# jihun1998/AO

Measured on AMD Instinct MI355X. Metric: points/sec fwd+bwd PTv2m2 S3DIS, higher is better.
Workload: dtype fp32

## Files before the change

### ao_amd/csrc/common.h

```cpp
#pragma once
#include <hip/hip_runtime.h>
#include <stdint.h>
#include <stdlib.h>

#include "../../include/ptv2_hip.h"

#define WAVE 64

#define PTV2_CHECK_LAUNCH()                         \
    do {                                            \
        if (hipGetLastError() != hipSuccess) return PTV2_ERR_LAUNCH; \
    } while (0)

#define RUN(call)                        \
    do {                                 \
        int rc_ = (call);                \
        if (rc_ != PTV2_OK) return rc_;  \
    } while (0)

static inline int divup(long long a, long long b) { return (int)((a + b - 1) / b); }

static constexpr size_t ptv2_align256(size_t v) { return (v + 255) & ~(size_t)255; }
struct PtvCarver {
    char *p; size_t off;
    char *take(size_t bytes) { char *r = p ? p + off : nullptr; off += ptv2_align256(bytes); return r; }
    template <class T> T *take_n(size_t count) { return (T *)take(sizeof(T) * count); }
};

static inline bool ptv2_env_set(const char *name) { return getenv(name) != nullptr; }
static inline bool ptv2_env_is(const char *name, char c) { const char *e = getenv(name); return e && e[0] == c; }

enum PtvKernelId {
    KID_KNN_QUERY = 0, KID_LOGITS_FWD, KID_SOFTMAX_ROWS, KID_AGG_TILE, KID_PEB_FWD, KID_PEB_BWD, KID_BWD_TILE,
    KID_BWD_ROWS, KID_BWD_GV, KID_LOGITS_BWD_ROWS, KID_LOGITS_BWD_GATHER, KID_LOGITS_BWD_PARAMS, KID_WGRAD,
    KID_BN_STATS, KID_BN_APPLY, KID_BN_BWD_REDUCE, KID_BN_BWD_APPLY, KID_SKINNY_FWD, KID_SKINNY_BWD, KID_ROWS_GEMM,  KID_BWD_POINT = KID_ROWS_GEMM + 8,
     KID_WGRAD_LDS = KID_BWD_POINT + 5 ,
    KID_WGRAD_GROUPED ,
    KID_FWD_POINT ,
    KID_LOGITS_BWD_FUSED ,
    KID_BN_BWD_APPLY_RES = KID_LOGITS_BWD_FUSED + 5 ,
    KID_BN_BWD_FINAPPLY ,
    KID_FWD_TILE ,
    KID_WGRAD_TILE = KID_FWD_TILE + 4 ,
    KID_BWD_TILE_K ,
    KID_AUG_POINTS = KID_BWD_TILE_K + 4 ,
    KID_COUNT
};
extern "C" int ptv2_profile_is_on(void);
int ptv2_profile_wants(int kid);
void ptv2_profile_begin(int kid, hipStream_t st);
void ptv2_profile_end(int kid, hipStream_t st, double algorithmic_bytes);
struct PtvScopedTimer {
    int kid; hipStream_t st; double bytes; bool on;
    PtvScopedTimer(int k, hipStream_t s, double b) : kid(k), st(s), bytes(b), on(ptv2_profile_wants(k) != 0) {
        if (on) ptv2_profile_begin(kid, st);
    }
    ~PtvScopedTimer() { if (on) ptv2_profile_end(kid, st, bytes); }
};

enum PtvGraphSlot { GRAPH_MODEL_FWD = 0, GRAPH_MODEL_BWD = 1, GRAPH_MODEL_FWD_PREFIX = 2, GRAPH_MODEL_FWD_REST = 3, GRAPH_SLOTS = 4 };
struct PtvGraphScope {
    void *st, *cap; int which, ring_entry; bool active; long long t0;
    PtvGraphScope(void *stream, int which, bool allow = true);
    void *stream() const { return cap; }
    int finish(int rc);
    ~PtvGraphScope();
    PtvGraphScope(const PtvGraphScope &) = delete;
    PtvGraphScope &operator=(const PtvGraphScope &) = delete;
};
int ptv2_graph_capturing(void);
int ptv2_profile_stamps(void);
int ptv2_zero_async(void *p, size_t bytes, hipStream_t st);

void ptv2_wgrad_defer_begin(void *arena, size_t bytes);
bool ptv2_wgrad_defer_active();
float *ptv2_wgrad_defer_alloc(size_t floats);
void ptv2_wgrad_defer_arm(bool on);
void ptv2_wgrad_defer_arm_rs(bool on);
bool ptv2_wgrad_defer_armed_rs();
struct PtvWgradArm {
    explicit PtvWgradArm(bool on) { ptv2_wgrad_defer_arm(on); }
    ~PtvWgradArm() { ptv2_wgrad_defer_arm(false); }
    PtvWgradArm(const PtvWgradArm &) = delete;
    PtvWgradArm &operator=(const PtvWgradArm &) = delete;
};
struct PtvWgradArmRs {
    explicit PtvWgradArmRs(bool on) { ptv2_wgrad_defer_arm_rs(on); }
    ~PtvWgradArmRs() { ptv2_wgrad_defer_arm_rs(false); }
    PtvWgradArmRs(const PtvWgradArmRs &) = delete;
    PtvWgradArmRs &operator=(const PtvWgradArmRs &) = delete;
};
int ptv2_wgrad_defer_flush(void *stream);
void ptv2_wgrad_defer_end();
size_t ptv2_wgrad_defer_table_bytes();

int ptv2_matmul_bf16(void);
void ptv2_set_matmul_bf16(int on);
struct PtvMatmulScope {
    int prev;
    explicit PtvMatmulScope(int on) : prev(ptv2_matmul_bf16()) { ptv2_set_matmul_bf16(on); }
    ~PtvMatmulScope() { ptv2_set_matmul_bf16(prev); }
};
typedef __bf16 ptv2_bf16x8 __attribute__((ext_vector_type(8)));
__device__ __forceinline__ ptv2_bf16x8 ptv2_pack_bf16(float4 lo, float4 hi) {
    ptv2_bf16x8 r;
    r[0] = (__bf16)lo.x; r[1] = (__bf16)lo.y; r[2] = (__bf16)lo.z; r[3] = (__bf16)lo.w;
    r[4] = (__bf16)hi.x; r[5] = (__bf16)hi.y; r[6] = (__bf16)hi.z; r[7] = (__bf16)hi.w;
    return r;
}

static __device__ __attribute__((aligned(16), unused)) float ptv2_zero_pad[1024];
template <class T>
__device__ __forceinline__ T ptv2_ld_or_zero(const T *p, bool ok) {
    return *(ok ? p : (const T *)ptv2_zero_pad);
}

#define PTV2_NUM_COUNTERS 64
enum PtvCounterSlot { CNT_LOGITS_FWD = 0, CNT_BP2, CNT_LOGITS_BWD_ROWS, CNT_CE, CNT_LOVASZ, CNT_BN_TILES = 16  };
unsigned *ptv2_stream_counters(hipStream_t st);

__device__ __forceinline__ float ref_d2(float qx, float qy, float qz, float x, float y, float z) {
    float dx = qx - x, dy = qy - y, dz = qz - z;
    return __builtin_fmaf(dz, dz, __builtin_fmaf(dx, dx, dy * dy));
}

__device__ __forceinline__ int seg_of(int pt, const int *__restrict__ offset, int b) {
    int lo = 0, hi = b - 1;
    while (lo < hi) {
        int mid = (lo + hi) >> 1;
        if (pt < offset[mid]) hi = mid; else lo = mid + 1;
    }
    return lo;
}

__device__ __forceinline__ int f2ord(float f) {
    int i = __float_as_int(f);
    return i >= 0 ? i : i ^ 0x7fffffff;
}
__device__ __forceinline__ float ord2f(int i) {
    return __int_as_float(i >= 0 ? i : i ^ 0x7fffffff);
}

__device__ __forceinline__ unsigned long long shfl_xor_u64(unsigned long long v, int m) {
    unsigned lo = (unsigned)v, hi = (unsigned)(v >> 32);
    lo = __shfl_xor(lo, m, WAVE);
    hi = __shfl_xor(hi, m, WAVE);
    return ((unsigned long long)hi << 32) | lo;
}

__device__ __forceinline__ int xcd_remap(int orig, int nwg) {
    int q = nwg >> 3, r = nwg & 7, x = orig & 7;
    return (x < r ? x * (q + 1) : r * (q + 1) + (x - r) * q) + (orig >> 3);
}
// ... 3 lines not shown
```

### ao_amd/csrc/graph.hip

```cpp
#include <algorithm>
#include <atomic>
#include <chrono>
#include <cstdio>
#include <cstdlib>
#include <mutex>
#include <unordered_map>

#include "common.h"

namespace {

struct SlotKey {
    int device;
    hipStream_t stream;
    int which;
    bool operator==(const SlotKey &o) const { return device == o.device && stream == o.stream && which == o.which; }
};
struct SlotKeyHash {
    size_t operator()(const SlotKey &k) const {
        return std::hash<void *>()((void *)k.stream) * 131u + (size_t)k.device * 7u + (size_t)k.which;
    }
};
constexpr int RING = 8;
struct Exec {
    hipGraphExec_t exec = nullptr;
    size_t nodes = 0;
    hipEvent_t done = nullptr;
    bool in_flight = false;
    unsigned long long seq = 0;
};
struct Slot {
    Exec ring[RING];
    unsigned long long launches = 0;
};
int pick_entry(Slot &slot) {
    int oldest = 0;
    for (int i = 0; i < RING; ++i) {
        Exec &e = slot.ring[i];
        if (e.in_flight && e.done && hipEventQuery(e.done) == hipSuccess) e.in_flight = false;
        if (!e.in_flight) return i;
        if (e.seq < slot.ring[oldest].seq) oldest = i;
    }
    (void)hipGetLastError();
    return oldest;
}
struct StreamKey {
    int device;
    hipStream_t stream;
    bool operator==(const StreamKey &o) const { return device == o.device && stream == o.stream; }
};
struct StreamKeyHash {
    size_t operator()(const StreamKey &k) const { return std::hash<void *>()((void *)k.stream) * 131u + (size_t)k.device; }
};
std::unordered_map<StreamKey, hipStream_t, StreamKeyHash> g_capture_streams;

std::mutex g_mu;
std::unordered_map<SlotKey, Slot, SlotKeyHash> g_slots;
std::unordered_map<StreamKey, hipEvent_t, StreamKeyHash> g_last_done;
std::atomic<int> g_mode{-1};
thread_local int g_inside = 0;

struct Stats {
    std::atomic<long long> scopes{0}, updated{0}, instantiated{0}, declined{0}, nodes{0};
    std::atomic<long long> capture_ns{0}, update_ns{0}, launch_ns{0}, wait_ns{0};
} g_stats;

long long now_ns() {
    return std::chrono::duration_cast<std::chrono::nanoseconds>(std::chrono::steady_clock::now().time_since_epoch()).count();
}

int mode() {
    int m = g_mode.load(std::memory_order_relaxed);
    if (m < 0) {
        m = ptv2_env_is("AO_AMD_GRAPH", '0') ? 0 : 1;
        g_mode.store(m, std::memory_order_relaxed);
    }
    return m;
}

}

int ptv2_graph_capturing(void) { return g_inside; }

namespace {
__global__ __launch_bounds__(256) void zero_kernel(float4 *__restrict__ p, long long n4, float *__restrict__ tail, int ntail) {
    const float4 z = make_float4(0.f, 0.f, 0.f, 0.f);
    for (long long i = (long long)blockIdx.x * 256 + threadIdx.x; i < n4; i += (long long)gridDim.x * 256) p[i] = z;
    if (blockIdx.x == 0 && (int)threadIdx.x < ntail) tail[threadIdx.x] = 0.f;
}
}

int ptv2_zero_async(void *p, size_t bytes, hipStream_t st) {
    if (bytes == 0) return PTV2_OK;
    if (!p || (bytes & 3) || ((uintptr_t)p & 15)) return PTV2_ERR_ARG;
    const long long n4 = (long long)(bytes >> 4);
    const int ntail = (int)((bytes & 15) >> 2);
    const int grid = (int)std::min<long long>(std::max<long long>((n4 + 255) / 256, 1), 2048);
    hipLaunchKernelGGL(zero_kernel, dim3(grid), dim3(256), 0, st, (float4 *)p, n4, (float *)p + 4 * n4, ntail);
    return PTV2_OK;
}

extern "C" int ptv2_graph_mode(int on) {
    const int prev = mode();
    if (on >= 0) g_mode.store(on ? 1 : 0, std::memory_order_relaxed);
    return prev;
}

extern "C" int ptv2_graph_stats(double *out, int reset) {
    if (out) {
        out[0] = (double)g_stats.scopes.load(); out[1] = (double)g_stats.updated.load();
        out[2] = (double)g_stats.instantiated.load(); out[3] = (double)g_stats.declined.load();
        out[4] = (double)g_stats.nodes.load(); out[5] = 1e-3 * (double)g_stats.capture_ns.load();
        out[6] = 1e-3 * (double)g_stats.update_ns.load(); out[7] = 1e-3 * (double)g_stats.launch_ns.load();
        out[8] = 1e-3 * (double)g_stats.wait_ns.load();
    }
    if (reset) {
        g_stats.scopes = 0; g_stats.updated = 0; g_stats.instantiated = 0; g_stats.declined = 0; g_stats.nodes = 0;
        g_stats.capture_ns = 0; g_stats.update_ns = 0; g_stats.launch_ns = 0; g_stats.wait_ns = 0;
    }
    return PTV2_OK;
}

extern "C" int ptv2_graph_reset(void) {
    std::lock_guard<std::mutex> lk(g_mu);
    for (auto &kv : g_slots)
        for (Exec &e : kv.second.ring) {
            if (e.in_flight && e.done) (void)hipEventSynchronize(e.done);
            if (e.exec) (void)hipGraphExecDestroy(e.exec);
            if (e.done) (void)hipEventDestroy(e.done);
        }
    g_slots.clear();
    g_last_done.clear();
    for (auto &kv : g_capture_streams) (void)hipStreamDestroy(kv.second);
    g_capture_streams.clear();
    return PTV2_OK;
}

PtvGraphScope::PtvGraphScope(void *stream, int which_, bool allow)
    : st(stream), cap(stream), which(which_), ring_entry(0), active(false), t0(0) {
    hipStream_t s = (hipStream_t)stream;
    if (!allow || !mode() || g_inside) { g_stats.declined++; return; }
    if (ptv2_profile_is_on() && !ptv2_profile_stamps()) { g_stats.declined++; return; }
    hipStreamCaptureStatus cs = hipStreamCaptureStatusNone;
    if (s != nullptr && (hipStreamIsCapturing(s, &cs) != hipSuccess || cs != hipStreamCaptureStatusNone)) {
        g_stats.declined++; (void)hipGetLastError(); return;
    }
    int device = 0;
    if (hipGetDevice(&device) != hipSuccess) { g_stats.declined++; return; }
    if (which == GRAPH_MODEL_FWD_PREFIX || which == GRAPH_MODEL_FWD) {
        if (!ptv2_env_is("AO_AMD_GRAPH_IDLE_EAGER", '0')) {
            hipEvent_t last = nullptr;
            {
                std::lock_guard<std::mutex> lk(g_mu);
                auto it = g_last_done.find(StreamKey{device, s});
                if (it != g_last_done.end()) last = it->second;
            }
            if (last && hipEventQuery(last) == hipSuccess) return;
            (void)hipGetLastError();
        }
    }
    hipStream_t c = nullptr;
    {
        std::lock_guard<std::mutex> lk(g_mu);
        auto it = g_capture_streams.find(StreamKey{device, s});
        if (it != g_capture_streams.end()) {
            c = it->second;
        } else {
            if (hipStreamCreateWithFlags(&c, hipStreamNonBlocking) != hipSuccess) { g_stats.declined++; (void)hipGetLastError(); return; }
            if (!ptv2_stream_counters(c) || hipStreamSynchronize(c) != hipSuccess) {
                (void)hipStreamDestroy(c); g_stats.declined++; return;
            }
            g_capture_streams[StreamKey{device, s}] = c;
        }
    }
    int entry = 0;
    {
        std::lock_guard<std::mutex> lk(g_mu);
        entry = pick_entry(g_slots[SlotKey{device, s, which}]);
    }
    t0 = now_ns();
    if (hipStreamBeginCapture(c, hipStreamCaptureModeRelaxed) != hipSuccess) { g_stats.declined++; (void)hipGetLastError(); return; }
    cap = (void *)c;
    active = true;
    g_inside = 1;
    g_stats.scopes++;
    ring_entry = entry;
    ptv2_profile_scope(which, 0, entry, RING);
}

int PtvGraphScope::finish(int rc) {
    if (!active) return rc;
    active = false;
    ptv2_profile_scope(which, 1, 0, RING);
    g_inside = 0;
    hipStream_t s = (hipStream_t)st;
    hipGraph_t g = nullptr;
    const hipError_t ec = hipStreamEndCapture((hipStream_t)cap, &g);
    const long long t1 = now_ns();
    g_stats.capture_ns += t1 - t0;
    if (ec != hipSuccess || !g) { (void)hipGetLastError(); if (g) (void)hipGraphDestroy(g); return rc != PTV2_OK ? rc : PTV2_ERR_LAUNCH; }
    if (rc != PTV2_OK) { (void)hipGraphDestroy(g); return rc; }
    int device = 0;
    (void)hipGetDevice(&device);
    size_t nodes = 0;
    (void)hipGraphGetNodes(g, nullptr, &nodes);
    int out = PTV2_OK;
    Exec *slot_p = nullptr;
    Slot *ring_p = nullptr;
    {
        std::lock_guard<std::mutex> lk(g_mu);
        Slot &ring = g_slots[SlotKey{device, s, which}];
        ring_p = &ring;
        slot_p = &ring.ring[ring_entry];
        slot_p->seq = ++ring.launches;
    }
    {
        Exec &slot = *slot_p;
        if (!slot.done && hipEventCreateWithFlags(&slot.done, hipEventDisableTiming | hipEventBlockingSync) != hipSuccess) slot.done = nullptr;
        if (slot.in_flight && slot.done) {
            const long long w0 = now_ns();
            (void)hipEventSynchronize(slot.done);
            g_stats.wait_ns += now_ns() - w0;
            slot.in_flight = false;
        }
        {
            static const int lead = [] { const char *e = getenv("AO_AMD_GRAPH_LEAD"); const int v = e ? atoi(e) : RING; return v < 1 ? 1 : (v > RING ? RING : v); }();
            if (lead < RING) {
                for (;;) {
                    int inflight = 0; Exec *oldest = nullptr;
                    for (int e2 = 0; e2 < RING; ++e2) {
                        Exec &o = ring_p->ring[e2];
                        if (&o == &slot || !o.in_flight || !o.done) continue;
                        if (hipEventQuery(o.done) == hipSuccess) { o.in_flight = false; continue; }
                        ++inflight;
                        if (!oldest || o.seq < oldest->seq) oldest = &o;
                    }
                    (void)hipGetLastError();
                    if (inflight < lead || !oldest) break;
                    const long long w0 = now_ns();
                    (void)hipEventSynchronize(oldest->done);
                    g_stats.wait_ns += now_ns() - w0;
                    oldest->in_flight = false;
                }
            }
        }
        const long long t1b = now_ns();
        bool ready = false;
        static const bool debug = ptv2_env_is("AO_AMD_GRAPH_DEBUG", '1');
        if (slot.exec && slot.nodes == nodes) {
            hipGraphExecUpdateResult res = hipGraphExecUpdateSuccess;
            hipGraphNode_t bad = nullptr;
            const hipError_t eu = hipGraphExecUpdate(slot.exec, g, &bad, &res);
            if (eu == hipSuccess && res == hipGraphExecUpdateSuccess) {
                ready = true;
                g_stats.updated++;
            } else {
                (void)hipGetLastError();
                if (debug) fprintf(stderr, "ptv2 graph: slot %d update failed rc %d result %d (%zu nodes)\n", which, (int)eu, (int)res, nodes);
            }
        } else if (debug && slot.exec) {
            fprintf(stderr, "ptv2 graph: slot %d node count %zu -> %zu\n", which, slot.nodes, nodes);
        }
        if (!ready) {
            if (slot.exec) { (void)hipGraphExecDestroy(slot.exec); slot.exec = nullptr; }
            if (hipGraphInstantiate(&slot.exec, g, nullptr, nullptr, 0) != hipSuccess) {
                (void)hipGetLastError();
                slot.exec = nullptr;
                out = PTV2_ERR_LAUNCH;
            } else {
                slot.nodes = nodes;
                g_stats.instantiated++;
                if (!ptv2_profile_is_on()) {
                    for (int e = 0; e < RING; ++e) {
                        Exec &o = ring_p->ring[e];
                        if (&o == &slot || o.exec || o.in_flight) continue;
                        if (hipGraphInstantiate(&o.exec, g, nullptr, nullptr, 0) != hipSuccess) { (void)hipGetLastError(); o.exec = nullptr; break; }
                        o.nodes = nodes;
                    }
                }
            }
        }
        const long long t2 = now_ns();
        g_stats.update_ns += t2 - t1b;
        if (out == PTV2_OK) {
            if (hipGraphLaunch(slot.exec, s) != hipSuccess) { (void)hipGetLastError(); out = PTV2_ERR_LAUNCH; }
            else if (slot.done && hipEventRecord(slot.done, s) == hipSuccess) {
                slot.in_flight = true;
                std::lock_guard<std::mutex> lk(g_mu);
                g_last_done[StreamKey{device, s}] = slot.done;
            }
            else if (hipStreamSynchronize(s) != hipSuccess) out = PTV2_ERR_LAUNCH;
            g_stats.launch_ns += now_ns() - t2;
            g_stats.nodes += (long long)nodes;
        }
    }
    (void)hipGraphDestroy(g);
    return out;
}

PtvGraphScope::~PtvGraphScope() {
    if (!active) return;
    ptv2_profile_scope(which, 1, 0, RING);
    g_inside = 0;
    hipGraph_t g = nullptr;
    (void)hipStreamEndCapture((hipStream_t)cap, &g);
    if (g) (void)hipGraphDestroy(g);
    (void)hipGetLastError();
}
```

### ao_amd/csrc/wgrad.hip

```cpp
#include <vector>

#include "dense_common.h"
#include "wgrad_job.h"

namespace dense {

using f32x4 = __attribute__((ext_vector_type(4))) float;
constexpr int WG_MT = 3, WG_TILE = 16 * WG_MT, WG_CHUNK = 256, WG_CHUNK_MIN = 128;

template <bool BF16>
__device__ __forceinline__ void wgrad_direct_tile(const int n, const int cout, const int cin, const int tiles_i,
                                                  const float *__restrict__ A, const long long ldy,
                                                  const float *__restrict__ B, const long long ldx, float *__restrict__ part,
                                                  const bool part_b, const int batch, const float *__restrict__ xs,
                                                  const float *__restrict__ xh, const int chunk, const int bx, const int by,
                                                  const int bz) {
    __shared__ float sRed[TPB / WAVE][WG_MT * WG_MT * 4 + WG_MT][WAVE + 1];
    const int lane = threadIdx.x & 63, wid = threadIdx.x >> 6;
    const int to = (by / tiles_i) * WG_TILE, ti = (by % tiles_i) * WG_TILE;
    const long long r0 = (long long)bx * chunk;
    const long long r1 = (r0 + chunk) < (long long)n ? (r0 + chunk) : (long long)n;
    const int lr = lane >> 4, lc = lane & 15;
    f32x4 acc[WG_MT][WG_MT];
    float bsum[WG_MT];
#pragma unroll
    for (int m = 0; m < WG_MT; ++m) {
        bsum[m] = 0.f;
#pragma unroll
        for (int t = 0; t < WG_MT; ++t) acc[m][t] = (f32x4){0.f, 0.f, 0.f, 0.f};
    }
    bool mo[WG_MT], mi[WG_MT];
    float xsc_[WG_MT], xsh_[WG_MT];
#pragma unroll
    for (int m = 0; m < WG_MT; ++m) {
        mo[m] = to + m * 16 + lc < cout;
        mi[m] = ti + m * 16 + lc < cin;
        xsc_[m] = (xs && mi[m]) ? xs[ti + m * 16 + lc] : 1.f;
        xsh_[m] = (xs && mi[m]) ? xh[ti + m * 16 + lc] : 0.f;
    }
    constexpr int U = 8;
    for (long long rb = r0 + 4 * wid; rb < r1; rb += 4 * (TPB / WAVE) * U) {
        float a[U][WG_MT], b[U][WG_MT];
#pragma unroll
        for (int u = 0; u < U; ++u) {
            const long long row = rb + (long long)u * 4 * (TPB / WAVE) + lr;
            const bool rok = row < r1;
#pragma unroll
            for (int m = 0; m < WG_MT; ++m) {
                a[u][m] = (rok && mo[m]) ? A[row * ldy + to + m * 16 + lc] : 0.f;
                b[u][m] = (rok && mi[m]) ? B[row * ldx + ti + m * 16 + lc] : 0.f;
            }
        }
        if (xs) {
#pragma unroll
            for (int u = 0; u < U; ++u)
#pragma unroll
                for (int m = 0; m < WG_MT; ++m) b[u][m] = fmaxf(__builtin_fmaf(b[u][m], xsc_[m], xsh_[m]), 0.f);
        }
        if constexpr (BF16) {
            ptv2_bf16x8 ab[WG_MT], bb[WG_MT];
#pragma unroll
            for (int m = 0; m < WG_MT; ++m) {
#pragma unroll
                for (int u = 0; u < U; ++u) {
                    bsum[m] += a[u][m];
                    ab[m][u] = (__bf16)a[u][m];
                    bb[m][u] = (__bf16)b[u][m];
                }
            }
#pragma unroll
            for (int m = 0; m < WG_MT; ++m)
#pragma unroll
                for (int t = 0; t < WG_MT; ++t)
                    acc[m][t] = __builtin_amdgcn_mfma_f32_16x16x32_bf16(ab[m], bb[t], acc[m][t], 0, 0, 0);
        } else {
#pragma unroll
            for (int u = 0; u < U; ++u)
#pragma unroll
                for (int m = 0; m < WG_MT; ++m) {
                    bsum[m] += a[u][m];
#pragma unroll
                    for (int t = 0; t < WG_MT; ++t)
// ... 116 lines not shown
    stash(0);
    __syncthreads();
    int buf = 0;
    for (long long rs = r0; rs < r1; rs += WL_ROWS, buf ^= 1) {
        const bool more = rs + WL_ROWS < r1;
        if (more) fetch(rs + WL_ROWS);
        const float *pa = sA + (size_t)buf * WL_ROWS * WG_TILE + (size_t)(wid * 16 + lr) * WG_TILE + lc;
        const float *pb = sB + (size_t)buf * WL_ROWS * WG_TILE + (size_t)(wid * 16 + lr) * WG_TILE + lc;
#pragma unroll
        for (int ks = 0; ks < 4; ++ks) {
            float a[WG_MT], b[WG_MT];
#pragma unroll
            for (int m = 0; m < WG_MT; ++m) {
                a[m] = pa[ks * 4 * WG_TILE + m * 16];
                b[m] = pb[ks * 4 * WG_TILE + m * 16];
            }
            if (xs) {
#pragma unroll
                for (int m = 0; m < WG_MT; ++m) b[m] = fmaxf(__builtin_fmaf(b[m], xsc_[m], xsh_[m]), 0.f);
            }
#pragma unroll
            for (int m = 0; m < WG_MT; ++m) {
                if constexpr (RS != 0) bsum[m] = __builtin_fmaf(a[m], sc_[ks], bsum[m]);
                else bsum[m] += a[m];
#pragma unroll
                for (int t = 0; t < WG_MT; ++t) acc[m][t] = __builtin_amdgcn_mfma_f32_16x16x4f32(a[m], b[t], acc[m][t], 0, 0, 0);
            }
        }
        if (more) {
            stash(buf ^ 1);
            __syncthreads();
        }
    }
    __syncthreads();
    float(*sRed)[WG_MT * WG_MT * 4 + WG_MT][WAVE + 1] = (float(*)[WG_MT * WG_MT * 4 + WG_MT][WAVE + 1]) wl_lds4;
#pragma unroll
    for (int m = 0; m < WG_MT; ++m) {
        float bs = bsum[m];
        bs += __shfl_xor(bs, 16, WAVE);
        bs += __shfl_xor(bs, 32, WAVE);
        sRed[wid][WG_MT * WG_MT * 4 + m][lane] = bs;
#pragma unroll
        for (int t = 0; t < WG_MT; ++t)
#pragma unroll
            for (int r = 0; r < 4; ++r) sRed[wid][(m * WG_MT + t) * 4 + r][lane] = acc[m][t][r];
    }
    __syncthreads();
    const size_t rec = (size_t)batch * cout * cin + (part_b ? (size_t)batch * cout : 0);
    float *p = part + (size_t)bx * rec + (size_t)bz * cout * cin;
    for (int e = threadIdx.x; e < WG_MT * WG_MT * 4 * WAVE; e += TPB) {
        const int q = e / WAVE, l = e - q * WAVE;
        const int mt = q / 4, r = q - mt * 4, m = mt / WG_MT, t = mt - m * WG_MT;
        const int o = to + m * 16 + (l >> 4) * 4 + r, i = ti + t * 16 + (l & 15);
        if (o < cout && i < cin) {
            float v = 0.f;
#pragma unroll
            for (int wv = 0; wv < TPB / WAVE; ++wv) v += sRed[wv][q][l];
            p[(size_t)o * cin + i] = v;
        }
    }
    if (part_b && ti == 0 && threadIdx.x < WG_TILE) {
        const int m = threadIdx.x >> 4, l = threadIdx.x & 15, o = to + threadIdx.x;
        if (o < cout) {
            float v = 0.f;
#pragma unroll
            for (int wv = 0; wv < TPB / WAVE; ++wv) v += sRed[wv][WG_MT * WG_MT * 4 + m][l];
            part[(size_t)bx * rec + (size_t)batch * cout * cin + (size_t)bz * cout + o] = v;
        }
    }
}

template <int RS>
__device__ __forceinline__ void wgrad_lds_job(const WgradJob &J, const int bx, const int by, const int bz) {
    const bool multi = J.count > 0;
    wgrad_lds_tile<RS>(J.n, J.cout, J.cin, J.tiles_i, multi ? J.mgY[bz] : J.gY + (long long)bz * J.sy, J.ldy,
                       multi ? J.mX[bz] : J.X + (long long)bz * J.sx, J.ldx, J.part, J.has_pb != 0, J.batch,
                       multi ? J.mxsc[bz] : nullptr, multi ? J.mxsh[bz] : nullptr, J.chunk, J.rowscale, J.lds_s, bx, by, bz);
}
template <int RS>
__global__ __launch_bounds__(TPB) void linear_wgrad_lds_kernel(WgradJob J) {
    wgrad_lds_job<RS>(J, (int)blockIdx.x, (int)blockIdx.y, (int)blockIdx.z);
}

constexpr int WGRAD_PACK = 8;
struct WgradJobPack { WgradJob j[WGRAD_PACK]; };
static_assert(sizeof(WgradJobPack) + 16 <= 4096, "the table writer's argument block must fit the 4 KB kernarg segment");
__global__ void wgrad_jobs_write_kernel(WgradJobPack pack, int count, WgradJob *table) {
    if ((int)threadIdx.x < count) table[threadIdx.x] = pack.j[threadIdx.x];
}

template <int RS>
__global__ __launch_bounds__(TPB) void linear_wgrad_lds_kernel_jobs(const WgradJob *__restrict__ jobs, int njobs) {
    int j = 0;
    while (j + 1 < njobs && (int)blockIdx.x >= jobs[j + 1].wg0) ++j;
    const WgradJob &J = jobs[j];
    const int local = (int)blockIdx.x - J.wg0;
    const int rest = local / J.chunks;
    wgrad_lds_job<RS>(J, local % J.chunks, rest % J.tiles, rest / J.tiles);
}

constexpr int GRP_I = 8;
__device__ __forceinline__ void grouped_wgrad_tile(const int n, const int c, const int g, const int gw, const int chunk,
                                                   const float *__restrict__ gY, const float *__restrict__ X,
                                                   const float *__restrict__ sw, float *__restrict__ part, const int rec,
                                                   const int bx, const int bg) {
    extern __shared__ float4 grp_lds4[];
    const int q = c >> 2, units = gw * q, R = max(1, TPB / units);
    const int tid = threadIdx.x, rs = tid / units, u = tid - rs * units;
    const bool active = rs < R;
    const int gl = u / q, qi = u - gl * q, grp = bg * gw + gl;
    const bool live = active && grp < g;
    float4 acc[GRP_I];
    float bacc[GRP_I];
#pragma unroll
    for (int i = 0; i < GRP_I; ++i) { acc[i] = make_float4(0.f, 0.f, 0.f, 0.f); bacc[i] = 0.f; }
    const long long r0 = (long long)bx * chunk, r1 = (r0 + chunk) < (long long)n ? (r0 + chunk) : (long long)n;
    if (live) {
        const float *xa = X + (size_t)grp * c + 4 * qi;
        const float *ya = gY + (size_t)grp * GRP_I;
        const float *sa = sw + grp;
        const size_t xs = (size_t)g * c;
        constexpr int U = 4;
        long long r = r0 + rs;
        for (; r + (long long)(U - 1) * R < r1; r += (long long)U * R) {
            float4 a[U], y0[U], y1[U];
            float s[U];
#pragma unroll
            for (int t = 0; t < U; ++t) {
                const size_t rr = (size_t)(r + (long long)t * R);
                a[t] = *(const float4 *)(xa + rr * xs);
                y0[t] = *(const float4 *)(ya + rr * c);
                y1[t] = *(const float4 *)(ya + rr * c + 4);
                s[t] = qi == 0 ? sa[rr * g] : 0.f;
            }
#pragma unroll
            for (int t = 0; t < U; ++t) {
                const float y[GRP_I] = {y0[t].x, y0[t].y, y0[t].z, y0[t].w, y1[t].x, y1[t].y, y1[t].z, y1[t].w};
#pragma unroll
                for (int i = 0; i < GRP_I; ++i) {
                    acc[i].x = __builtin_fmaf(y[i], a[t].x, acc[i].x); acc[i].y = __builtin_fmaf(y[i], a[t].y, acc[i].y);
                    acc[i].z = __builtin_fmaf(y[i], a[t].z, acc[i].z); acc[i].w = __builtin_fmaf(y[i], a[t].w, acc[i].w);
                    bacc[i] = __builtin_fmaf(y[i], s[t], bacc[i]);
                }
            }
        }
        for (; r < r1; r += R) {
            const size_t rr = (size_t)r;
            const float4 a = *(const float4 *)(xa + rr * xs), y0 = *(const float4 *)(ya + rr * c), y1 = *(const float4 *)(ya + rr * c + 4);
            const float sv = qi == 0 ? sa[rr * g] : 0.f;
            const float y[GRP_I] = {y0.x, y0.y, y0.z, y0.w, y1.x, y1.y, y1.z, y1.w};
#pragma unroll
            for (int i = 0; i < GRP_I; ++i) {
                acc[i].x = __builtin_fmaf(y[i], a.x, acc[i].x); acc[i].y = __builtin_fmaf(y[i], a.y, acc[i].y);
                acc[i].z = __builtin_fmaf(y[i], a.z, acc[i].z); acc[i].w = __builtin_fmaf(y[i], a.w, acc[i].w);
                bacc[i] = __builtin_fmaf(y[i], sv, bacc[i]);
            }
        }
    }
    float4 *sAcc = grp_lds4;
    float *sB = (float *)(sAcc + (size_t)R * GRP_I * units);
    if (active) {
#pragma unroll
        for (int i = 0; i < GRP_I; ++i) {
            sAcc[((size_t)rs * GRP_I + i) * units + u] = acc[i];
            if (qi == 0) sB[((size_t)rs * GRP_I + i) * gw + gl] = bacc[i];
        }
    }
    __syncthreads();
    if (rs == 0 && grp < g) {
        float *p = part + (size_t)bx * rec;
#pragma unroll
        for (int i = 0; i < GRP_I; ++i) {
            float4 v = sAcc[(size_t)i * units + u];
            for (int t = 1; t < R; ++t) {
                const float4 w = sAcc[((size_t)t * GRP_I + i) * units + u];
                v.x += w.x; v.y += w.y; v.z += w.z; v.w += w.w;
            }
            *(float4 *)(p + ((size_t)grp * GRP_I + i) * c + 4 * qi) = v;
            if (qi == 0) {
                float b = sB[(size_t)i * gw + gl];
                for (int t = 1; t < R; ++t) b += sB[((size_t)t * GRP_I + i) * gw + gl];
                p[(size_t)g * GRP_I * c + (size_t)grp * GRP_I + i] = b;
            }
        }
    }
}
inline size_t grouped_lds_bytes(int c, int gw) {
    const int units = gw * (c >> 2), R = std::max(1, TPB / units);
    return sizeof(float4) * (size_t)R * GRP_I * units + sizeof(float) * (size_t)R * GRP_I * gw;
}
__global__ __launch_bounds__(TPB) void grouped_wgrad_kernel(WgradJob J) {
    const int bx = (int)blockIdx.x % J.chunks, bg = (int)blockIdx.x / J.chunks;
    grouped_wgrad_tile(J.n, J.cin, J.batch, J.gw, J.chunk, J.gY, J.X, J.rowscale, J.part, J.rec, bx, bg);
}
__global__ __launch_bounds__(TPB) void grouped_wgrad_kernel_jobs(const WgradJob *__restrict__ jobs, int njobs) {
    int j = 0;
    while (j + 1 < njobs && (int)blockIdx.x >= jobs[j + 1].wg0) ++j;
    const WgradJob &J = jobs[j];
    const int local = (int)blockIdx.x - J.wg0;
    grouped_wgrad_tile(J.n, J.cin, J.batch, J.gw, J.chunk, J.gY, J.X, J.rowscale, J.part, J.rec, local % J.chunks, local / J.chunks);
}

template <bool BF16>
__global__ __launch_bounds__(TPB) void linear_wgrad_kernel_jobs(const WgradJob *__restrict__ jobs, int njobs) {
    int j = 0;
    while (j + 1 < njobs && (int)blockIdx.x >= jobs[j + 1].wg0) ++j;
    const WgradJob &J = jobs[j];
    const int local = (int)blockIdx.x - J.wg0;
    const int rest = local / J.chunks;
    wgrad_direct_job<BF16>(J, local % J.chunks, rest % J.tiles, rest / J.tiles);
}

__global__ __launch_bounds__(256) void wgrad_jobs_finalize_kernel(const WgradJob *__restrict__ jobs, int njobs, int total) {
    __shared__ double s_sum[3][64];
    const int sidx = blockIdx.x * 256 + threadIdx.x;
    int j = 0;
    while (j + 1 < njobs && (int)blockIdx.x * 256 >= jobs[j + 1].fin0) ++j;
    const WgradJob &J = jobs[j];
    const int lanes = J.fin_lanes, local = sidx - J.fin0;
    const int rg = lanes == 1 ? 0 : (int)threadIdx.x >> 6;
    const int col = lanes == 1 ? local : (local >> 8) * 64 + ((int)threadIdx.x & 63);
    const int nblk = J.chunks;
    const size_t len = (size_t)J.rec;
    const float *part = J.part;
    const bool ok = col < J.rec;
    double a0 = 0.0, a1 = 0.0, a2 = 0.0, a3 = 0.0;
    if (ok) {
        int b = rg;
        for (; b + 3 * lanes < nblk; b += 4 * lanes) {
            a0 += (double)part[(size_t)b * len + col];
            a1 += (double)part[(size_t)(b + lanes) * len + col];
            a2 += (double)part[(size_t)(b + 2 * lanes) * len + col];
            a3 += (double)part[(size_t)(b + 3 * lanes) * len + col];
        }
        for (; b < nblk; b += lanes) a0 += (double)part[(size_t)b * len + col];
    }
    double acc = (a0 + a1) + (a2 + a3);
    if (lanes != 1) {
        if (rg > 0) s_sum[rg - 1][threadIdx.x & 63] = acc;
        __syncthreads();
        if (rg > 0) return;
        acc = (acc + s_sum[0][threadIdx.x]) + (s_sum[1][threadIdx.x] + s_sum[2][threadIdx.x]);
    }
    if (!ok) return;
    const float v = (float)acc;
    const int wlen = J.cout * J.cin, wtot = J.batch * wlen;
    if (J.count > 0) {
        if (col < wtot) {
            const int p = col / wlen;
            J.mdW[p][col - p * wlen] = v;
        } else {
            const int r = col - wtot, p = r / J.cout;
            if (J.mdb[p]) J.mdb[p][r - p * J.cout] = v;
        }
    } else if (col < wtot) {
        J.dW[col] = v;
    } else if (J.db) {
        J.db[col - wtot] = v;
    }
}

static bool wgrad_lds_ok(const void *a, long long ldy, long long sy, const void *b, long long ldx, long long sx) {
    return ((uintptr_t)a % 16 == 0) && ((uintptr_t)b % 16 == 0) && ldy % 4 == 0 && ldx % 4 == 0 && sy % 4 == 0 && sx % 4 == 0;
}
static bool wgrad_lds_shape_ok(int cout, int cin) { return cout % 4 == 0 && cin % 4 == 0; }
constexpr size_t WL_LDS_BYTES = sizeof(float) * std::max<size_t>(4 * (size_t)WL_ROWS * WG_TILE,
                                                                 (size_t)(TPB / WAVE) * (WG_MT * WG_MT * 4 + WG_MT) * (WAVE + 1));

}

using namespace dense;

extern "C" size_t dense_workspace_bytes(int n, int cout, int cin) {
    const size_t chunks = (size_t)(n + WG_CHUNK_MIN - 1) / WG_CHUNK_MIN + 1;
    const size_t wg = sizeof(float) * chunks * ((size_t)cout * cin + cout);
    const size_t bn = sizeof(float) * (size_t)MAX_BLK * 2 * (size_t)std::max(cout, cin);
    return ptv2_align256(std::max(wg, bn)) + 1024;
}

static int wg_chunk(int n, int tiles, bool filed = false) {
    const int target = filed ? 256 : 768;
    const int chunks = std::max(1, target / std::max(1, tiles));
    const long long rows = ((long long)n + chunks - 1) / chunks;
    long long chunk = std::max<long long>(WG_CHUNK, (rows + 127) / 128 * 128);
    if (tiles > 1) {
        int guard = 0;
        while ((((long long)n + chunk - 1) / chunk) % 8 == 0 && ((long long)n + chunk - 1) / chunk > 1 && guard++ < 16) chunk += 128;
    }
    return (int)std::min<long long>(chunk, 1 << 20);
}

namespace {
enum WgradForm { WF_LDS = 0, WF_LDS_RS, WF_DIRECT, WF_DIRECT_BF16, WF_GROUPED, WF_RECOMPUTE, WGRAD_FORMS };
constexpr int wgrad_kid(WgradForm f) {
    return f == WF_RECOMPUTE ? KID_WGRAD_TILE : f == WF_GROUPED ? KID_WGRAD_GROUPED : (f == WF_LDS || f == WF_LDS_RS) ? KID_WGRAD_LDS : KID_WGRAD;
}
struct WgradCall {
    WgradJob J;
    WgradForm form;
    double bytes;
    size_t posrel;
};

struct WgradDefer {
    bool active = false;
    bool armed = false;
    bool armed_rs = false;
    char *arena = nullptr;
    size_t cap = 0, used = 0;
    std::vector<WgradJob> jobs[WGRAD_FORMS];
    double bytes[WGRAD_FORMS] = {};
};
thread_local WgradDefer g_wdefer;
constexpr int WGRAD_MAX_JOBS = 64;
constexpr size_t WGRAD_TABLE_BYTES = ptv2_align256(sizeof(WgradJob) * WGRAD_MAX_JOBS);

bool may_file(bool rs) { return g_wdefer.active && (rs ? g_wdefer.armed_rs : g_wdefer.armed); }

bool wgrad_configure() {
    static const bool ok = [] {
        const void *kernels[4] = {(const void *)linear_wgrad_lds_kernel<0>, (const void *)linear_wgrad_lds_kernel<1>,
                                  (const void *)linear_wgrad_lds_kernel_jobs<0>, (const void *)linear_wgrad_lds_kernel_jobs<1>};
        bool all = true;
        for (const void *k : kernels)
            all = hipFuncSetAttribute(k, hipFuncAttributeMaxDynamicSharedMemorySize, (int)WL_LDS_BYTES) == hipSuccess && all;
        return all;
    }();
    return ok;
}
}

void ptv2_wgrad_defer_begin(void *arena, size_t bytes) {
    WgradDefer &D = g_wdefer;
    for (int f = 0; f < WGRAD_FORMS; ++f) { D.jobs[f].clear(); D.bytes[f] = 0.0; }
    D.armed = D.armed_rs = false;
    D.active = arena != nullptr && bytes > WGRAD_FORMS * WGRAD_TABLE_BYTES;
    D.arena = (char *)arena;
    D.cap = bytes;
    D.used = WGRAD_FORMS * WGRAD_TABLE_BYTES;
}
bool ptv2_wgrad_defer_active() { return g_wdefer.active; }
void ptv2_wgrad_defer_end() {
    g_wdefer.active = g_wdefer.armed = g_wdefer.armed_rs = false;
    for (auto &j : g_wdefer.jobs) j.clear();
}
void ptv2_wgrad_defer_arm(bool on) { g_wdefer.armed = on && g_wdefer.active; }
void ptv2_wgrad_defer_arm_rs(bool on) { g_wdefer.armed_rs = on && g_wdefer.active; }
bool ptv2_wgrad_defer_armed_rs() { return may_file(true); }
size_t ptv2_wgrad_defer_table_bytes() { return WGRAD_FORMS * WGRAD_TABLE_BYTES; }
float *ptv2_wgrad_defer_alloc(size_t floats) {
    WgradDefer &D = g_wdefer;
    const size_t bytes = ptv2_align256(sizeof(float) * floats);
    if (!D.active || D.used + bytes > D.cap) return nullptr;
    float *p = (float *)(D.arena + D.used);
    D.used += bytes;
    return p;
}
int ptv2_wgrad_defer_flush(void *stream) {
    WgradDefer &D = g_wdefer;
    if (!D.active) return PTV2_OK;
    hipStream_t st = (hipStream_t)stream;
    if (!wgrad_configure()) return PTV2_ERR_LAUNCH;
    for (int f = 0; f < WGRAD_FORMS; ++f) {
        const WgradForm form = (WgradForm)f;
        std::vector<WgradJob> &jobs = D.jobs[form];
        if (jobs.empty()) continue;
        WgradJob *table = (WgradJob *)(D.arena + (size_t)form * WGRAD_TABLE_BYTES);
        const int njobs = (int)jobs.size();
        const bool row_pieces = form == WF_GROUPED || form == WF_RECOMPUTE;
        std::stable_sort(jobs.begin(), jobs.end(), [row_pieces](const WgradJob &a, const WgradJob &b) {
            const long long wa = (long long)a.chunk * (row_pieces ? a.gw * a.cin : 1), wb = (long long)b.chunk * (row_pieces ? b.gw * b.cin : 1);
            return wa > wb;
        });
        int wgs = 0, fin = 0;
        long long pos_wgs = 0;
        bool pos_all = form == WF_RECOMPUTE;
        for (WgradJob &J : jobs) {
            if (form == WF_RECOMPUTE) {
                J.ldy = pos_wgs;
                pos_wgs += ((long long)J.n * 16 + 255) / 256;
                pos_all = pos_all && J.mX[0] != nullptr;
            }
            J.wg0 = wgs; J.fin0 = fin;
            J.fin_lanes = J.chunks > 32 ? 4 : 1;
            wgs += J.wgs;
            fin += J.fin_lanes == 1 ? (J.rec + 255) / 256 * 256 : (J.rec + 63) / 64 * 256;
        }
        for (int at = 0; at < njobs; at += WGRAD_PACK) {
            WgradJobPack pack;
            const int cnt = std::min(WGRAD_PACK, njobs - at);
            for (int i = 0; i < WGRAD_PACK; ++i) pack.j[i] = jobs[(size_t)std::min(at + i, njobs - 1)];
            hipLaunchKernelGGL(wgrad_jobs_write_kernel, dim3(1), dim3(64), 0, st, pack, cnt, table + at);
        }
        {
            PtvScopedTimer t(wgrad_kid(form), st, D.bytes[form]);
            const dim3 grid((unsigned)wgs), block(TPB);
            const WgradJob *tab = table;
            switch (form) {
                case WF_LDS: hipLaunchKernelGGL(linear_wgrad_lds_kernel_jobs<0>, grid, block, WL_LDS_BYTES, st, tab, njobs); break;
                case WF_LDS_RS: hipLaunchKernelGGL(linear_wgrad_lds_kernel_jobs<1>, grid, block, WL_LDS_BYTES, st, tab, njobs); break;
                case WF_DIRECT: hipLaunchKernelGGL(linear_wgrad_kernel_jobs<false>, grid, block, 0, st, tab, njobs); break;
                case WF_DIRECT_BF16: hipLaunchKernelGGL(linear_wgrad_kernel_jobs<true>, grid, block, 0, st, tab, njobs); break;
                case WF_GROUPED: {
                    size_t lds = 0;
                    for (const WgradJob &J : jobs) lds = std::max(lds, grouped_lds_bytes(J.cin, J.gw));
                    hipLaunchKernelGGL(grouped_wgrad_kernel_jobs, grid, block, lds, st, tab, njobs);
                    break;
                }
                default:
                    if (gva_wgrad_tile_launch_jobs(tab, njobs, wgs, pos_all ? (int)pos_wgs : 0, st) != PTV2_OK) return PTV2_ERR_LAUNCH;
            }
        }
        hipLaunchKernelGGL(wgrad_jobs_finalize_kernel, dim3((unsigned)((fin + 255) / 256)), dim3(256), 0, st,
                           (const WgradJob *)table, njobs, fin);
        jobs.clear();
        D.bytes[form] = 0.0;
    }
    PTV2_CHECK_LAUNCH();
    return PTV2_OK;
}

struct MapWgradMulti {
    float *dW[6], *db[6];
    int count, wlen, cout;
    explicit MapWgradMulti(const WgradJob &J) : count(J.count), wlen(J.cout * J.cin), cout(J.cout) {
        for (int i = 0; i < 6; ++i) { dW[i] = J.mdW[i]; db[i] = J.mdb[i]; }
    }
    __device__ void operator()(int e, double v) const {
        const int wtot = count * wlen;
        if (e < wtot) {
            const int b = e / wlen;
            dW[b][e - b * wlen] = (float)v;
        } else {
            const int r = e - wtot, b = r / cout;
            if (db[b]) db[b][r - b * cout] = (float)v;
        }
    }
};

namespace gva {
template <> struct RiderOf<MapWgradMulti> {
    static constexpr bool ok = true;
    static PtvRider make(const MapWgradMulti &m) {
        PtvRider r{};
        r.kind = RIDER_WGRADN;
        for (int i = 0; i < 6; ++i) { r.p[i] = i < m.count ? m.dW[i] : nullptr; r.p[6 + i] = i < m.count ? m.db[i] : nullptr; }
        r.i0 = m.wlen; r.i1 = m.cout; r.i2 = m.count;
        return r;
    }
};
}

static int wgrad_submit(WgradCall &C, bool file, void *workspace, size_t workspace_bytes, void *stream) {
    WgradDefer &D = g_wdefer;
    WgradJob &J = C.J;
    if (file && (int)D.jobs[C.form].size() < WGRAD_MAX_JOBS) {
        float *keep = ptv2_wgrad_defer_alloc((size_t)J.chunks * J.rec);
        float *pos = keep && C.posrel ? ptv2_wgrad_defer_alloc(C.posrel) : nullptr;
        if (keep && (pos || !C.posrel)) {
            J.part = keep;
            if (pos) J.mX[0] = pos;
            D.jobs[C.form].push_back(J);
            D.bytes[C.form] += C.bytes;
            return PTV2_OK;
        }
    }
    const size_t fit = workspace ? workspace_bytes / (sizeof(float) * (size_t)J.rec) : 0;
    if (C.form == WF_RECOMPUTE && fit >= 1 && fit < (size_t)J.chunks) (void)gva_wgrad_tile_plan(&J, (int)fit);
    if (fit < (size_t)J.chunks) return PTV2_ERR_WORKSPACE;
    if (!wgrad_configure()) return PTV2_ERR_LAUNCH;
    hipStream_t st = (hipStream_t)stream;
    J.part = (float *)workspace;
    {
        PtvScopedTimer t(wgrad_kid(C.form), st, C.bytes);
        const dim3 grid(J.chunks, J.tiles, J.batch), block(TPB);
        switch (C.form) {
            case WF_LDS: hipLaunchKernelGGL(linear_wgrad_lds_kernel<0>, grid, block, WL_LDS_BYTES, st, J); break;
            case WF_LDS_RS: hipLaunchKernelGGL(linear_wgrad_lds_kernel<1>, grid, block, WL_LDS_BYTES, st, J); break;
            case WF_DIRECT: hipLaunchKernelGGL(linear_wgrad_kernel<false>, grid, block, 0, st, J); break;
            case WF_DIRECT_BF16: hipLaunchKernelGGL(linear_wgrad_kernel<true>, grid, block, 0, st, J); break;
            case WF_GROUPED:
                hipLaunchKernelGGL(grouped_wgrad_kernel, dim3((unsigned)J.wgs), block, grouped_lds_bytes(J.cin, J.gw), st, J);
                break;
            default:
                if (gva_wgrad_tile_launch_one(J, st) != PTV2_OK) return PTV2_ERR_LAUNCH;
        }
    }
    if (J.count > 0) launch_finalize(st, (const float *)J.part, J.chunks, J.rec, MapWgradMulti(J));
    else if (J.has_pb) launch_finalize(st, (const float *)J.part, J.chunks, J.rec, gva::MapSplit2<float>{J.dW, J.db, J.batch * J.cout * J.cin});
    else launch_finalize(st, (const float *)J.part, J.chunks, J.rec, gva::MapVec<float>{J.dW});
    PTV2_CHECK_LAUNCH();
    return PTV2_OK;
}

static void plan_tiles(WgradJob &J, int n, int cout, int cin, int batch, bool filed) {
    J.n = n; J.cout = cout; J.cin = cin; J.batch = batch;
    J.tiles_i = (cin + WG_TILE - 1) / WG_TILE;
    J.tiles = (cout + WG_TILE - 1) / WG_TILE * J.tiles_i;
    J.chunk = wg_chunk(n, J.tiles * batch, filed);
    J.chunks = (n + J.chunk - 1) / J.chunk;
// ... 148 lines not shown
```

Baseline: 12.79 million.

## Stage wgrad job table in pinned host memory and merge per-form finalize launches

The deferred weight-gradient flush now builds one combined job table for all forms. When a backward graph is being captured, that table is copied into a per-ring-entry pinned host staging buffer and written to the device by a single copy kernel, instead of several 8-job kernarg-packed writer launches. The separate finalize kernels per form are merged into one launch, which finds each block's job by binary search. To make reuse of the staging buffer safe, the graph scope now synchronises on the previous launch of the same ring entry before capturing. That wait can stall the host, and pos_all now depends on a flag computed across all forms.

```diff
diff --git a/ao_amd/csrc/common.h b/ao_amd/csrc/common.h
--- a/ao_amd/csrc/common.h
+++ b/ao_amd/csrc/common.h
@@ -69,6 +69,7 @@
     PtvGraphScope &operator=(const PtvGraphScope &) = delete;
 };
 int ptv2_graph_capturing(void);
+void *ptv2_graph_stage(size_t bytes);
 int ptv2_profile_stamps(void);
 int ptv2_zero_async(void *p, size_t bytes, hipStream_t st);
 
diff --git a/ao_amd/csrc/graph.hip b/ao_amd/csrc/graph.hip
--- a/ao_amd/csrc/graph.hip
+++ b/ao_amd/csrc/graph.hip
@@ -32,6 +32,8 @@
 struct Slot {
     Exec ring[RING];
     unsigned long long launches = 0;
+    void *stage = nullptr;
+    size_t stage_bytes = 0;
 };
 int pick_entry(Slot &slot) {
     int oldest = 0;
@@ -59,6 +61,8 @@
 std::unordered_map<StreamKey, hipEvent_t, StreamKeyHash> g_last_done;
 std::atomic<int> g_mode{-1};
 thread_local int g_inside = 0;
+thread_local char *g_stage = nullptr;
+thread_local size_t g_stage_bytes = 0, g_stage_used = 0;
 
 struct Stats {
     std::atomic<long long> scopes{0}, updated{0}, instantiated{0}, declined{0}, nodes{0};
@@ -81,6 +85,14 @@
 }
 
 int ptv2_graph_capturing(void) { return g_inside; }
+
+void *ptv2_graph_stage(size_t bytes) {
+    bytes = ptv2_align256(bytes);
+    if (!g_inside || !g_stage || g_stage_used + bytes > g_stage_bytes) return nullptr;
+    void *p = g_stage + g_stage_used;
+    g_stage_used += bytes;
+    return p;
+}
 
 namespace {
 __global__ __launch_bounds__(256) void zero_kernel(float4 *__restrict__ p, long long n4, float *__restrict__ tail, int ntail) {
@@ -129,6 +141,8 @@
             if (e.exec) (void)hipGraphExecDestroy(e.exec);
             if (e.done) (void)hipEventDestroy(e.done);
         }
+    for (auto &kv : g_slots)
+        if (kv.second.stage) (void)hipHostFree(kv.second.stage);
     g_slots.clear();
     g_last_done.clear();
     for (auto &kv : g_capture_streams) (void)hipStreamDestroy(kv.second);
@@ -174,12 +188,34 @@
         }
     }
     int entry = 0;
+    Slot *slot = nullptr;
     {
         std::lock_guard<std::mutex> lk(g_mu);
-        entry = pick_entry(g_slots[SlotKey{device, s, which}]);
+        slot = &g_slots[SlotKey{device, s, which}];
+        entry = pick_entry(*slot);
+    }
+    g_stage = nullptr;
+    if (which == GRAPH_MODEL_BWD) {
+        Exec *ex = &slot->ring[entry];
+        if (ex->in_flight && ex->done) {
+            const long long w0 = now_ns();
+            (void)hipEventSynchronize(ex->done);
+            g_stats.wait_ns += now_ns() - w0;
+            ex->in_flight = false;
+        }
+        if (!slot->stage) {
+            const size_t want = 2 * ptv2_wgrad_defer_table_bytes();
+            if (hipHostMalloc(&slot->stage, RING * want, hipHostMallocDefault) == hipSuccess) slot->stage_bytes = want;
+            else { slot->stage = nullptr; (void)hipGetLastError(); }
+        }
+        if (slot->stage) {
+            g_stage = (char *)slot->stage + (size_t)entry * slot->stage_bytes;
+            g_stage_bytes = slot->stage_bytes;
+            g_stage_used = 0;
+        }
     }
     t0 = now_ns();
-    if (hipStreamBeginCapture(c, hipStreamCaptureModeRelaxed) != hipSuccess) { g_stats.declined++; (void)hipGetLastError(); return; }
+    if (hipStreamBeginCapture(c, hipStreamCaptureModeRelaxed) != hipSuccess) { g_stats.declined++; g_stage = nullptr; (void)hipGetLastError(); return; }
     cap = (void *)c;
     active = true;
     g_inside = 1;
@@ -193,6 +229,7 @@
     active = false;
     ptv2_profile_scope(which, 1, 0, RING);
     g_inside = 0;
+    g_stage = nullptr;
     hipStream_t s = (hipStream_t)st;
     hipGraph_t g = nullptr;
     const hipError_t ec = hipStreamEndCapture((hipStream_t)cap, &g);
@@ -302,6 +339,7 @@
     if (!active) return;
     ptv2_profile_scope(which, 1, 0, RING);
     g_inside = 0;
+    g_stage = nullptr;
     hipGraph_t g = nullptr;
     (void)hipStreamEndCapture((hipStream_t)cap, &g);
     if (g) (void)hipGraphDestroy(g);
diff --git a/ao_amd/csrc/wgrad.hip b/ao_amd/csrc/wgrad.hip
--- a/ao_amd/csrc/wgrad.hip
+++ b/ao_amd/csrc/wgrad.hip
@@ -1,3 +1,4 @@
+#include <cstring>
 #include <vector>
 
 #include "dense_common.h"
@@ -280,10 +281,14 @@
     wgrad_lds_job<RS>(J, (int)blockIdx.x, (int)blockIdx.y, (int)blockIdx.z);
 }
 
+__global__ __launch_bounds__(256) void wgrad_jobs_write_kernel(const uint4 *__restrict__ staged, uint4 *__restrict__ table, int pieces) {
+    const int i = (int)blockIdx.x * 256 + (int)threadIdx.x;
+    if (i < pieces) table[i] = staged[i];
+}
 constexpr int WGRAD_PACK = 8;
 struct WgradJobPack { WgradJob j[WGRAD_PACK]; };
 static_assert(sizeof(WgradJobPack) + 16 <= 4096, "the table writer's argument block must fit the 4 KB kernarg segment");
-__global__ void wgrad_jobs_write_kernel(WgradJobPack pack, int count, WgradJob *table) {
+__global__ void wgrad_jobs_write_pack_kernel(WgradJobPack pack, int count, WgradJob *table) {
     if ((int)threadIdx.x < count) table[threadIdx.x] = pack.j[threadIdx.x];
 }
 
@@ -413,7 +418,11 @@
     __shared__ double s_sum[3][64];
     const int sidx = blockIdx.x * 256 + threadIdx.x;
     int j = 0;
-    while (j + 1 < njobs && (int)blockIdx.x * 256 >= jobs[j + 1].fin0) ++j;
+    for (int hi = njobs; hi - j > 1;) {
+        const int mid = (j + hi) >> 1;
+        if ((int)blockIdx.x * 256 >= jobs[mid].fin0) j = mid;
+        else hi = mid;
+    }
     const WgradJob &J = jobs[j];
     const int lanes = J.fin_lanes, local = sidx - J.fin0;
     const int rg = lanes == 1 ? 0 : (int)threadIdx.x >> 6;
@@ -507,6 +516,7 @@
     char *arena = nullptr;
     size_t cap = 0, used = 0;
     std::vector<WgradJob> jobs[WGRAD_FORMS];
+    std::vector<WgradJob> table;
     double bytes[WGRAD_FORMS] = {};
 };
 thread_local WgradDefer g_wdefer;
@@ -559,61 +569,75 @@
     if (!D.active) return PTV2_OK;
     hipStream_t st = (hipStream_t)stream;
     if (!wgrad_configure()) return PTV2_ERR_LAUNCH;
+    std::vector<WgradJob> &all = D.table;
+    all.clear();
+    int first[WGRAD_FORMS], wgs[WGRAD_FORMS] = {}, fin = 0;
+    long long pos_wgs = 0;
+    bool pos_all = true;
     for (int f = 0; f < WGRAD_FORMS; ++f) {
         const WgradForm form = (WgradForm)f;
         std::vector<WgradJob> &jobs = D.jobs[form];
-        if (jobs.empty()) continue;
-        WgradJob *table = (WgradJob *)(D.arena + (size_t)form * WGRAD_TABLE_BYTES);
-        const int njobs = (int)jobs.size();
+        first[f] = (int)all.size();
         const bool row_pieces = form == WF_GROUPED || form == WF_RECOMPUTE;
         std::stable_sort(jobs.begin(), jobs.end(), [row_pieces](const WgradJob &a, const WgradJob &b) {
             const long long wa = (long long)a.chunk * (row_pieces ? a.gw * a.cin : 1), wb = (long long)b.chunk * (row_pieces ? b.gw * b.cin : 1);
             return wa > wb;
         });
-        int wgs = 0, fin = 0;
-        long long pos_wgs = 0;
-        bool pos_all = form == WF_RECOMPUTE;
         for (WgradJob &J : jobs) {
             if (form == WF_RECOMPUTE) {
                 J.ldy = pos_wgs;
                 pos_wgs += ((long long)J.n * 16 + 255) / 256;
                 pos_all = pos_all && J.mX[0] != nullptr;
             }
-            J.wg0 = wgs; J.fin0 = fin;
+            J.wg0 = wgs[f]; J.fin0 = fin;
             J.fin_lanes = J.chunks > 32 ? 4 : 1;
-            wgs += J.wgs;
+            wgs[f] += J.wgs;
             fin += J.fin_lanes == 1 ? (J.rec + 255) / 256 * 256 : (J.rec + 63) / 64 * 256;
-        }
-        for (int at = 0; at < njobs; at += WGRAD_PACK) {
+            all.push_back(J);
+        }
+    }
+    const int total = (int)all.size();
+    if (total == 0) return PTV2_OK;
+    WgradJob *table = (WgradJob *)D.arena;
+    const size_t image = sizeof(WgradJob) * (size_t)total, pieces = (image + 15) / 16;
+    static_assert(WGRAD_TABLE_BYTES % 16 == 0, "the table's last 16-byte piece lies inside its room");
+    if (void *staged = ptv2_graph_stage(16 * pieces)) {
+        memcpy(staged, all.data(), image);
+        hipLaunchKernelGGL(wgrad_jobs_write_kernel, dim3((unsigned)((pieces + 255) / 256)), dim3(256), 0, st, (const uint4 *)staged,
+                           (uint4 *)table, (int)pieces);
+    } else {
+        for (int at = 0; at < total; at += WGRAD_PACK) {
             WgradJobPack pack;
-            const int cnt = std::min(WGRAD_PACK, njobs - at);
-            for (int i = 0; i < WGRAD_PACK; ++i) pack.j[i] = jobs[(size_t)std::min(at + i, njobs - 1)];
-            hipLaunchKernelGGL(wgrad_jobs_write_kernel, dim3(1), dim3(64), 0, st, pack, cnt, table + at);
-        }
-        {
-            PtvScopedTimer t(wgrad_kid(form), st, D.bytes[form]);
-            const dim3 grid((unsigned)wgs), block(TPB);
-            const WgradJob *tab = table;
-            switch (form) {
-                case WF_LDS: hipLaunchKernelGGL(linear_wgrad_lds_kernel_jobs<0>, grid, block, WL_LDS_BYTES, st, tab, njobs); break;
-                case WF_LDS_RS: hipLaunchKernelGGL(linear_wgrad_lds_kernel_jobs<1>, grid, block, WL_LDS_BYTES, st, tab, njobs); break;
-                case WF_DIRECT: hipLaunchKernelGGL(linear_wgrad_kernel_jobs<false>, grid, block, 0, st, tab, njobs); break;
-                case WF_DIRECT_BF16: hipLaunchKernelGGL(linear_wgrad_kernel_jobs<true>, grid, block, 0, st, tab, njobs); break;
-                case WF_GROUPED: {
-                    size_t lds = 0;
-                    for (const WgradJob &J : jobs) lds = std::max(lds, grouped_lds_bytes(J.cin, J.gw));
-                    hipLaunchKernelGGL(grouped_wgrad_kernel_jobs, grid, block, lds, st, tab, njobs);
-                    break;
-                }
-                default:
-                    if (gva_wgrad_tile_launch_jobs(tab, njobs, wgs, pos_all ? (int)pos_wgs : 0, st) != PTV2_OK) return PTV2_ERR_LAUNCH;
-            }
-        }
-        hipLaunchKernelGGL(wgrad_jobs_finalize_kernel, dim3((unsigned)((fin + 255) / 256)), dim3(256), 0, st,
-                           (const WgradJob *)table, njobs, fin);
-        jobs.clear();
-        D.bytes[form] = 0.0;
-    }
+            const int cnt = std::min(WGRAD_PACK, total - at);
+            for (int i = 0; i < WGRAD_PACK; ++i) pack.j[i] = all[(size_t)std::min(at + i, total - 1)];
+            hipLaunchKernelGGL(wgrad_jobs_write_pack_kernel, dim3(1), dim3(64), 0, st, pack, cnt, table + at);
+        }
+    }
+    for (int f = 0; f < WGRAD_FORMS; ++f) {
+        const WgradForm form = (WgradForm)f;
+        const int njobs = (int)D.jobs[form].size();
+        if (njobs == 0) continue;
+        PtvScopedTimer t(wgrad_kid(form), st, D.bytes[form]);
+        const dim3 grid((unsigned)wgs[f]), block(TPB);
+        const WgradJob *tab = table + first[f];
+        switch (form) {
+            case WF_LDS: hipLaunchKernelGGL(linear_wgrad_lds_kernel_jobs<0>, grid, block, WL_LDS_BYTES, st, tab, njobs); break;
+            case WF_LDS_RS: hipLaunchKernelGGL(linear_wgrad_lds_kernel_jobs<1>, grid, block, WL_LDS_BYTES, st, tab, njobs); break;
+            case WF_DIRECT: hipLaunchKernelGGL(linear_wgrad_kernel_jobs<false>, grid, block, 0, st, tab, njobs); break;
+            case WF_DIRECT_BF16: hipLaunchKernelGGL(linear_wgrad_kernel_jobs<true>, grid, block, 0, st, tab, njobs); break;
+            case WF_GROUPED: {
+                size_t lds = 0;
+                for (const WgradJob &J : D.jobs[form]) lds = std::max(lds, grouped_lds_bytes(J.cin, J.gw));
+                hipLaunchKernelGGL(grouped_wgrad_kernel_jobs, grid, block, lds, st, tab, njobs);
+                break;
+            }
+            default:
+                if (gva_wgrad_tile_launch_jobs(tab, njobs, wgs[f], pos_all ? (int)pos_wgs : 0, st) != PTV2_OK) return PTV2_ERR_LAUNCH;
+        }
+    }
+    hipLaunchKernelGGL(wgrad_jobs_finalize_kernel, dim3((unsigned)((fin + 255) / 256)), dim3(256), 0, st, (const WgradJob *)table,
+                       total, fin);
+    for (int f = 0; f < WGRAD_FORMS; ++f) { D.jobs[f].clear(); D.bytes[f] = 0.0; }
     PTV2_CHECK_LAUNCH();
     return PTV2_OK;
 }
```

Result: no change. 12.90 million (median of 6 runs) (+0.9%).
